# Xiongda337/fpm-OpenCV

Hardware: AMD Instinct MI355X
Metric: LED-updates/sec (patch·LED/s), 256² patch × 293 LEDs; 1/2/4/8 GPU (higher is better)
Workload: dtype f32

## Files before the change

### fpm-opencv_amd/csrc/fpm_fused.hip

```cpp
#include <hip/hip_runtime.h>

#include <vector>

#include "dft16.hpp"
#include "fft_lds.hpp"
#include "fpm_state.hpp"
#include "fused256.hpp"
#include "fused_common.hpp"
#include "fused_sync.hpp"
#include "launch.hpp"
#include "ledtab.hpp"
#include "tilemax.hpp"
#include "update.hpp"

namespace fpm {

constexpr int n_parts(int ks) { return ks == 1 ? 2 : ks; }
constexpr int part_cols(int ks) { return fz::NP / n_parts(ks); }

template <int NT>
struct FzCfg {
    static_assert(NT == 512, "512 threads per workgroup");
    static constexpr int NG = NT / 16;
    static constexpr int RPG = fz::NROWS / NG;
    static constexpr int NW = NT / 64;
    static constexpr int XT = XTILE;
};

template <int NT, int KS, bool GAIN>
__global__ void __launch_bounds__(NT, 1) k_fused_iteration(FusedArgs a) {
    using namespace fz;
    using C = FzCfg<NT>;
    constexpr int NG = C::NG, RPG = C::RPG, NW = C::NW;
    ClockProbe probe;
    probe.start();
    static_assert(KS == 1 || KS == 2 || KS == 4, "one workgroup per patch, or split mode with 2 / 4");
    static_assert(6 * RPG * 16 <= C::XT, "pupil numerators are parked in the group's exchange tile");
    constexpr int NPARTS = n_parts(KS), TH = part_cols(KS), TLD = TH + 1;
    extern __shared__ __attribute__((aligned(16))) float2 sm[];
    const int nrows = NROWS + a.n_tail_rows;
    float2 *scr_all = sm;
    float2 *th = scr_all + NG * C::XT;
    float2 *tw2 = th + (nrows + 2) * TLD;
    float2 *tw = tw2 + 256;
    float2 *tailX = tw + 256;
    float2 *tailF = tailX + MAXTAIL;
    float *red = (float *)(tailF + MAXTAIL);
    int *sig = (int *)(red + 48);
    int2 *tpx = (int2 *)(sig + 96);
    int *tky = (int *)(tpx + MAXTAIL);
    float *tmx = (float *)(tky + MAXTAILROWS);
    unsigned *dirty = (unsigned *)(tmx + a.band.nbt);
    int *ccnt = (int *)(dirty + ((a.band.nbt + 31) >> 5));

    const DevState &st = a.st;
    const int tid = threadIdx.x, g = tid >> 4, t = tid & 15, gg = (tid >> 4) & 3;
    const int xrd = exch_rbase(t);
    const int lane = tid & 63, w = tid >> 6;
    constexpr bool split = KS > 1;
    const int hown = split ? (int)((blockIdx.x >> 3) % KS) : -1;
    const int b = split ? (int)((blockIdx.x / (8 * KS)) * 8 + (blockIdx.x & 7)) : (int)blockIdx.x;
    if (b >= st.B) return;
    const int hb = hown < 0 ? 0 : hown, he = hown < 0 ? NPARTS : hown + 1;
    float2 *xch = split ? a.xch + (size_t)b * xch_patch_elems(KS) : nullptr;
    int *flg = split ? a.flags + KS * b : nullptr;
    int *xccs = split ? a.flags + KS * st.B + 1 + KS * b : nullptr;
    const int R = st.r, NB = st.nb, L = st.L;
    float2 *scr = scr_all + g * C::XT;
    const int nwords = (a.band.nbt + 31) >> 5;

    if (tid == 0) {
#pragma unroll
        for (int i = 0; i < MAXTAIL; ++i) tpx[i] = a.tail_px[i];
#pragma unroll
        for (int i = 0; i < MAXTAILROWS; ++i) tky[i] = a.tail_ky[i];
    }
    for (int i = tid; i < 256; i += NT) {
        tw[i] = a.tw[i];
        tw2[i] = a.tw[((i >> 4) * (i & 15)) & 255];
    }
    for (int i = tid; i < 96; i += NT) {
        const int ky = i - KYOFF;
        int s = -1;
        if (ky >= -R && ky <= R) {
            if (ky >= a.ky_lo && ky < a.ky_lo + a.n_fft_rows) s = ky - a.ky_lo;
#pragma unroll
            for (int q = 0; q < MAXTAILROWS; ++q)
                if (q < a.n_tail_rows && a.tail_ky[q] == ky) s = NROWS + q;
        }
        sig[i] = s;
    }
    auto band_dy = [&](int k) { return (int)(((float)k + 0.5f) * a.band.rnbx); };
    auto band_gtile = [&](int k) {
        const int dy = band_dy(k);
        return (a.band.bty0 + dy) * st.ntx + a.band.btx0 + (k - dy * a.band.nbx);
    };
    float *tmax_g = st.tmax + (size_t)b * st.ntx * st.nty;
    unsigned *dirty_g = st.tdirty + (size_t)b * ((st.ntx * st.nty + 31) / 32);
    for (int k = tid; k < a.band.nbt; k += NT) tmx[k] = tmax_g[band_gtile(k)];
    for (int i = tid; i < nwords; i += NT) dirty[i] = dirty_g[i];

    float2 *spec = st.spec + (size_t)b * L * L;
    float2 *pup = st.pupil + (size_t)b * NB * NB;
    int kyr[RPG];
    bool ron[RPG];
    float2 P[RPG][6];
    unsigned inmask[RPG];
#pragma unroll
    for (int j = 0; j < RPG; ++j) {
        kyr[j] = a.ky_lo + g + NG * j;
        ron[j] = g + NG * j < a.n_fft_rows;
        inmask[j] = 0;
#pragma unroll
        for (int s = 0; s < 6; ++s) {
            const int kx = slot_kx(t, s);
            const bool in = ron[j] && (kyr[j] * kyr[j] + kx * kx <= R * R);
            inmask[j] |= (in ? 1u : 0u) << s;
            P[j][s] = in ? pup[(kyr[j] + R) * NB + kx + R] : make_float2(0.f, 0.f);
        }
    }
    int2 *ltl = a.ledtab_off >= 0 ? (int2 *)((char *)sm + a.ledtab_off) : nullptr;
    const LedTab lt{ltl, a.order, a.x0, a.y0, NP / 2};
    if (ltl) lt.fill(ltl, a.n_order, tid, NT);
    __syncthreads();
    const int zoff = nrows * TLD;
    int roff[6];
#pragma unroll
    for (int s = 0; s < 6; ++s) {
        const int sg = sig[slot_kx(t, s) + KYOFF];
        roff[s] = sg >= 0 ? sg * TLD : zoff;
    }
    for (int i = tid; i < TLD; i += NT) th[zoff + i] = make_float2(0.f, 0.f);
    const bool towner = tid < a.n_tail_px;
    const int2 tp = towner ? tpx[tid] : make_int2(0, 0);
    float2 Pt = towner ? pup[(tp.x + R) * NB + tp.y + R] : make_float2(0.f, 0.f);
    float2 NPt = make_float2(0.f, 0.f), Ot = make_float2(0.f, 0.f);
    float pm = st.pmax[b];
    auto pm_of_red = [&]() {
        float pm2 = red[32];
#pragma unroll
        for (int i = 1; i < NW; ++i) pm2 = fmaxf(pm2, red[32 + i]);
        return sqrtf(pm2);
    };
    bool pupil_done = false;
    bool local = false;
    const __amdgpu_buffer_rsrc_t rx =
        __builtin_amdgcn_make_buffer_rsrc(xch, 0, split ? xch_patch_elems(KS) * (int)sizeof(float2) : 0, 0x00020000);
    const __amdgpu_buffer_rsrc_t rf = __builtin_amdgcn_make_buffer_rsrc(flg, 0, split ? KS * (int)sizeof(int) : 0, 0x00020000);
    const __amdgpu_buffer_rsrc_t rs =
        __builtin_amdgcn_make_buffer_rsrc(split ? st.spec + (size_t)b * L * L : nullptr, 0,
                                          split ? L * L * (int)sizeof(float2) : 0, 0x00020000);
    if (split) {
        if (tid == 0) {
            const int mine = xcc_id() + 1;
            __hip_atomic_store(xccs + hown, mine, __ATOMIC_RELAXED, __HIP_MEMORY_SCOPE_AGENT);
            bool same = true;
#pragma unroll
            for (int p = 0; p < KS; ++p) {
                if (p == hown) continue;
                int other = 0;
                for (int spins = 0; (other = __hip_atomic_load(xccs + p, __ATOMIC_RELAXED,
                                                               __HIP_MEMORY_SCOPE_AGENT)) == 0; ++spins) {
                    if (spins > (1 << 23) ||
                        __hip_atomic_load(a.abort_flag, __ATOMIC_RELAXED, __HIP_MEMORY_SCOPE_AGENT)) {
                        __hip_atomic_store(a.abort_flag, 1, __ATOMIC_RELAXED, __HIP_MEMORY_SCOPE_AGENT);
                        break;
                    }
                    __builtin_amdgcn_s_sleep(2);
                }
                same = same && other == mine;
            }
            ccnt[1] = same;
        }
        __syncthreads();
        local = ccnt[1] != 0;
        __syncthreads();
    }
    typedef unsigned u32x2_t __attribute__((ext_vector_type(2)));
    const int lane_off = tid * (int)sizeof(float2);
    auto xst = [&](int slot, float2 v) {
        const u32x2_t d = __builtin_bit_cast(u32x2_t, v);
        if (local) __builtin_amdgcn_raw_buffer_store_b64(d, rx, lane_off, slot * (int)sizeof(float2), 0);
        else __builtin_amdgcn_raw_buffer_store_b64(d, rx, lane_off, slot * (int)sizeof(float2), 16);
    };
    auto xld = [&](int slot) {
        return __builtin_bit_cast(
            float2, local ? __builtin_amdgcn_raw_buffer_load_b64(rx, lane_off, slot * (int)sizeof(float2), kAuxL2Volatile)
                          : __builtin_amdgcn_raw_buffer_load_b64(rx, lane_off, slot * (int)sizeof(float2),
                                                                 (int)(16u | (1u << 31))));
    };
    auto sst = [&](float2 *p, float2 v) {
        if (split && !local) {
            const int off = (int)((p - (st.spec + (size_t)b * L * L)) * (int)sizeof(float2));
            __builtin_amdgcn_raw_buffer_store_b64(__builtin_bit_cast(u32x2_t, v), rs, off, 0, 16);
        } else {
            *p = v;
        }
    };
    const float epsn = st.eps * (float)(NP * NP);
    const float epsn_im = st.eps_im * (float)(NP * NP);
    __syncthreads();

    FPM_STAMPS_BEGIN()
    auto window = [&](int itn) {
        const LedPos p = lt.at(itn);
        return spec + (unsigned)(p.yc * L + p.xc);
    };
    auto soff = [](int s) { return 16 * fz::SK[s] - (s >= 3 ? fz::NP : 0); };
    auto ldO = [&](const float2 *sr, int j, int s) {
        const float2 *lr = sr + (kyr[j] * L + t);
        return ((inmask[j] >> s) & 1) ? lr[soff(s)] : make_float2(0.f, 0.f);
    };
    float2 Opre[RPG][6];
    if (a.n_order > 0) {
        const float2 *sr = window(0);
#pragma unroll
        for (int j = 0; j < RPG; ++j)
#pragma unroll
            for (int s = 0; s < 6; ++s) Opre[j][s] = ldO(sr, j, s);
        if (towner) Ot = sr[tp.x * L + tp.y];
    }
    for (int it = 0; it < a.n_order; ++it) {
        const LedPos lp = lt.at(it);
        const int led = lp.led, xc = lp.xc, yc = lp.yc;
        float2 *srow = spec + (unsigned)(yc * L + xc);
        const uint16_t *Ib = a.meas + ((size_t)led * st.B + b) * NP * NP;
        const float gl = fused_gain<GAIN>(st, led, b);

        if (towner) tailX[tid] = pout(pmul(pin(Ot), pin(Pt)));
        __syncthreads();
        FPM_STAMP(0)

        float2 v[16], r[16];
        float2 F[RPG][6];
        bool aborted = false;
#pragma unroll 1
        for (int h = hb; h < he; ++h) {
            Tw wt;
            wt.load(tw2, t);
            constexpr int NBLK = TH / 4;
            auto colx = [&](int r8) { return (r8 & 15) + 16 * gg + 64 * (r8 >> 4); };
            auto ldI = [&](int xl, uint4 (&n)[2]) {
                const uint4 *ip = (const uint4 *)(Ib + ((xl + TH * h) * 16 + t) * 16);
#pragma unroll
                for (int i = 0; i < 2; ++i) n[i] = ld_stream(ip + i);
            };
            float2 X[RPG][6];
#pragma unroll
            for (int j = 0; j < RPG; ++j)
#pragma unroll
                for (int s = 0; s < 6; ++s) X[j][s] = pout(pmul(pin(Opre[j][s]), pin(P[j][s])));
#pragma unroll
            for (int j = 0; j < RPG; ++j) {
                if (!ron[j]) continue;
#pragma unroll
                for (int k = 0; k < 16; ++k) v[k] = make_float2(0.f, 0.f);
#pragma unroll
                for (int s = 0; s < 6; ++s) v[SK[s]] = X[j][s];
                idft256_in6(v, r, scr, wt, t, xrd);
                float2 *row = th + (g + NG * j) * TLD + t;
                if constexpr (NPARTS == 2) {
                    if (h == 0) {
#pragma unroll
                        for (int m = 0; m < 8; ++m) row[16 * m] = r[m];
                    } else {
#pragma unroll
                        for (int m = 0; m < 8; ++m) row[16 * m] = r[8 + m];
                    }
                } else {
                    if (h == 0) {
#pragma unroll
                        for (int m = 0; m < 4; ++m) row[16 * m] = r[m];
                    } else if (h == 1) {
#pragma unroll
                        for (int m = 0; m < 4; ++m) row[16 * m] = r[4 + m];
                    } else if (h == 2) {
#pragma unroll
                        for (int m = 0; m < 4; ++m) row[16 * m] = r[8 + m];
                    } else {
#pragma unroll
                        for (int m = 0; m < 4; ++m) row[16 * m] = r[12 + m];
                    }
                }
            }
            FPM_STAMP(7)
            for (int idx = tid; tid < NT / 2 && idx < a.n_tail_rows * TH; idx += NT / 2) {
                const int q = idx / TH, xl = idx - q * TH, x = xl + TH * h;
                const int p0 = a.tail_row_p0[q], np_ = a.tail_row_np[q];
                const int ti = (x * (a.tail_row_kx0[q] + NP)) & (NP - 1);
                pf2 wa = pin(tw[ti]), wb = pin(tw[(ti + x) & (NP - 1)]);
                const pf2 wstep = pin(tw[(2 * x) & (NP - 1)]);
                pf2 s2 = {0.f, 0.f}, s3 = {0.f, 0.f};
                int p = 0;
                for (; p + 1 < np_; p += 2) {
                    s2 += pmulc(pin(tailX[p0 + p]), wa);
                    s3 += pmulc(pin(tailX[p0 + p + 1]), wb);
                    wa = pmul(wa, wstep);
                    wb = pmul(wb, wstep);
                }
                if (p < np_) s2 += pmulc(pin(tailX[p0 + p]), wa);
                th[(NROWS + q) * TLD + xl] = pout(s2 + s3);
            }
            if (tid == 0) *ccnt = NW;
            __syncthreads();
            FPM_STAMP(1)

            float2 tin[6];
#pragma unroll
            for (int s = 0; s < 6; ++s) tin[s] = th[roff[s] + colx(w)];
            int r8 = w;
#pragma unroll 1
            for (;;) {
                const int xl = colx(r8);
                uint4 cI[2];
                int nx = 0;
                if (lane == 0) nx = atomicAdd(ccnt, 1);
                nx = __builtin_amdgcn_readfirstlane(nx);
                ldI(xl, cI);
#pragma unroll
                for (int k = 0; k < 16; ++k) v[k] = make_float2(0.f, 0.f);
#pragma unroll
                for (int s = 0; s < 6; ++s) v[SK[s]] = tin[s];
                idft256_in6(v, r, scr, wt, t, xrd);
                {
                    const int xn = colx(nx < NBLK ? nx : r8);
#pragma unroll
                    for (int s = 0; s < 6; ++s) tin[s] = th[roff[s] + xn];
                }
                const unsigned iw[8] = {cI[0].x, cI[0].y, cI[0].z, cI[0].w, cI[1].x, cI[1].y, cI[1].z, cI[1].w};
#pragma unroll
                for (int m2 = 0; m2 < 16; ++m2) {
                    const float Iv = (float)((m2 & 1) ? (iw[m2 >> 1] >> 16) : (iw[m2 >> 1] & 0xffffu));
                    const pf2 tt = pin(r[m2]) + (pf2){epsn, epsn_im};
                    const float mag2 = __builtin_fmaf(tt.x, tt.x, tt.y * tt.y);
                    const float sc = amp_scale(mag2, Iv);
                    v[m2] = pout(pin(r[m2]) * sc);
                }
                float2 o[6];
                dft256_out6(v, o, scr, wt, t, xrd);
#pragma unroll
                for (int s = 0; s < 6; ++s) th[roff[s] + (roff[s] == zoff ? TLD : 0) + xl] = o[s];
                if (nx >= NBLK) break;
                r8 = nx;
            }
            FPM_STAMP(10)
            __syncthreads();
            FPM_STAMP(2)

#pragma unroll
            for (int j = 0; j < RPG; ++j)
#pragma unroll
                for (int s = 0; s < 6; ++s) Opre[j][s] = ldO(srow, j, s);
#pragma unroll
            for (int j = 0; j < RPG; ++j) {
                if (!ron[j]) {
#pragma unroll
                    for (int s = 0; s < 6; ++s) F[j][s] = make_float2(0.f, 0.f);
                    continue;
                }
                float2 o[6];
                row_dft_part<NPARTS>(th + (g + NG * j) * TLD + t, v, o, scr, wt, t, xrd, h);
#pragma unroll
                for (int s = 0; s < 6; ++s) F[j][s] = h == hb ? o[s] : cadd(F[j][s], o[s]);
            }
            FPM_STAMP(8)
            for (int pp = g; g < NG / 2 && pp < a.n_tail_px; pp += NG / 2) {
                const int2 px = tpx[pp];
                const float2 *row = th + sig[px.x + KYOFF] * TLD;
                pf2 s2p = {0.f, 0.f};
                pf2 wk = pin(tw[((t + TH * h) * (px.y + NP)) & (NP - 1)]);
                const pf2 wstep = pin(tw[(16 * (px.y + NP)) & (NP - 1)]);
#pragma unroll
                for (int m = 0; m < TH / 16; ++m) {
                    s2p += pmul(pin(row[t + 16 * m]), wk);
                    if (m < TH / 16 - 1) wk = pmul(wk, wstep);
                }
                float2 s2 = pout(s2p);
                s2.x = row16_sum(s2.x);
                s2.y = row16_sum(s2.y);
                if (t == 0) tailF[pp] = h != hb ? cadd(tailF[pp], s2) : s2;
            }
            __syncthreads();
            FPM_STAMP(3)
        }
        if (split) {
            const int par = it & 1;
            const int mine = (hown * 2 + par) * kXchHalf;
            if (it < a.stall_led || a.stall_led < 0 || hown != KS - 1) {
#pragma unroll
                for (int j = 0; j < RPG; ++j)
#pragma unroll
                    for (int s = 0; s < 6; ++s)
                        if ((inmask[j] >> s) & 1) xst(mine + (j * 6 + s) * NT, F[j][s]);
                if (tid < a.n_tail_px) xst(mine + kXchTF, tailF[tid]);
                FPM_STAMP(11)
                handoff_publish(flg + hown, it + 1, local);
            }
            if (!handoff_wait<KS>(flg, hown, it + 1, a.abort_flag, ccnt + 1, local, rf)) {
                aborted = true;
                break;
            }
            FPM_STAMP(12)
            float2 ox[KS > 1 ? KS - 1 : 1][RPG][6];
#pragma unroll
            for (int q = 0; q < KS - 1; ++q) {
                const int pp = q < hown ? q : q + 1;
                const int base = (pp * 2 + par) * kXchHalf;
#pragma unroll
                for (int j = 0; j < RPG; ++j)
#pragma unroll
                    for (int s = 0; s < 6; ++s) {
                        const bool in = (inmask[j] >> s) & 1;
                        ox[q][j][s] = in ? xld(base + (j * 6 + s) * NT) : make_float2(0.f, 0.f);
                    }
            }
#pragma unroll
            for (int j = 0; j < RPG; ++j)
#pragma unroll
                for (int s = 0; s < 6; ++s) {
                    float2 acc = make_float2(0.f, 0.f);
#pragma unroll
                    for (int p = 0; p < KS; ++p) {
                        const float2 lo = ox[p < KS - 1 ? p : KS - 2][j][s], hi = ox[p > 0 ? p - 1 : 0][j][s];
                        const float2 o = p == hown ? F[j][s] : p < hown ? lo : hi;
                        acc = p == 0 ? o : cadd(acc, o);
                    }
                    F[j][s] = acc;
                }
            if (tid < a.n_tail_px) {
                float2 acc = make_float2(0.f, 0.f);
#pragma unroll
                for (int p = 0; p < KS; ++p) {
                    const float2 o = p == hown ? tailF[tid] : xld(((p * 2 + par) * kXchHalf) + kXchTF);
                    acc = p == 0 ? o : cadd(acc, o);
                }
                tailF[tid] = acc;
            }
        }

        unsigned *tmu = (unsigned *)tmx;
        auto note = [&](int py, int px, float ao, float an) {
            const int ti = ((py >> 4) - a.band.bty0) * a.band.nbx + ((px >> 4) - a.band.btx0);
            const unsigned cur = tmu[ti];
            if (an < ao && cur <= __float_as_uint(ao)) atomicOr(&dirty[ti >> 5], 1u << (ti & 31));
            if (__float_as_uint(an) > cur) atomicMax(&tmu[ti], __float_as_uint(an));
        };
        if (it > 0) pm = pm_of_red();
#pragma unroll
        for (int j = 0; j < RPG; ++j)
#pragma unroll
            for (int s = 0; s < 6; ++s) {
                float2 num = make_float2(0.f, 0.f);
                if ((inmask[j] >> s) & 1) {
                    float oa;
                    const float2 nv = slot_update<GAIN>(F[j][s], Opre[j][s], P[j][s], pm, gl, st, num, oa);
                    sst(srow + (kyr[j] * L + t) + soff(s), nv);
                    note(yc + kyr[j], xc + slot_kx(t, s), oa, cmag(nv));
                }
                scr[(j * 6 + s) * 16 + t] = num;
            }
        if (towner) {
            float oa;
            const float2 nv = slot_update<GAIN>(tailF[tid], Ot, Pt, pm, gl, st, NPt, oa);
            sst(srow + tp.x * L + tp.y, nv);
            note(yc + tp.x, xc + tp.y, oa, cmag(nv));
        }
        FPM_STAMP(9)
        __syncthreads();
        if (it + 1 < a.n_order) {
            const float2 *sr = window(it + 1);
#pragma unroll
            for (int j = 0; j < RPG; ++j)
#pragma unroll
                for (int s = 0; s < 6; ++s) Opre[j][s] = ldO(sr, j, s);
            if (towner) Ot = sr[tp.x * L + tp.y];
        }
        FPM_STAMP(4)

        float cm = 0.f, dm = 0.f;
        for (int k = tid; k < a.band.nbt; k += NT) {
            const bool d = tile_dirty(dirty, k);
            if (d) dm = fmaxf(dm, tmx[k]);
            else cm = fmaxf(cm, tmx[k]);
        }
        cm = wave_max_nonneg(cm);
        dm = wave_max_nonneg(dm);
        if (lane == 0) {
            red[w] = cm;
            red[16 + w] = dm;
        }
        __syncthreads();
        cm = red[0];
        dm = red[16];
#pragma unroll
        for (int i = 1; i < NW; ++i) {
            cm = fmaxf(cm, red[i]);
            dm = fmaxf(dm, red[16 + i]);
        }
        float omax = cm;
        if (dm > cm) {
            for (int k = w; k < a.band.nbt; k += NW) {
                if (!tile_dirty(dirty, k) || !(tmx[k] > cm)) continue;
                const int ty = a.band.bty0 + band_dy(k), tx = a.band.btx0 + k - band_dy(k) * a.band.nbx;
                float2 e[4];
#pragma unroll
                for (int jj = 0; jj < 4; ++jj) {
                    const int pp = lane + 64 * jj;
                    e[jj] = spec[(unsigned)((ty * 16 + (pp >> 4)) * L + tx * 16 + (pp & 15))];
                }
                float mm = 0.f;
#pragma unroll
                for (int jj = 0; jj < 4; ++jj) mm = fmaxf(mm, cmag(e[jj]));
                mm = wave_max_nonneg(mm);
                if (lane == 0) {
                    tmx[k] = mm;
                    atomicAnd(&dirty[k >> 5], ~(1u << (k & 31)));
                }
            }
            __syncthreads();
            float m2 = 0.f;
            for (int k = tid; k < a.band.nbt; k += NT)
                if (!tile_dirty(dirty, k)) m2 = fmaxf(m2, tmx[k]);
            m2 = wave_max_nonneg(m2);
            __syncthreads();
            if (lane == 0) red[w] = m2;
            __syncthreads();
            omax = red[0];
#pragma unroll
            for (int i = 1; i < NW; ++i) omax = fmaxf(omax, red[i]);
        }
        FPM_STAMP(5)
        const float rom = 1.0f / omax;
        float pmx = 0.f;
#pragma unroll
        for (int j = 0; j < RPG; ++j)
#pragma unroll
            for (int s = 0; s < 6; ++s) {
                const float2 n = scr[(j * 6 + s) * 16 + t];
                P[j][s] = make_float2(P[j][s].x + n.x * rom, P[j][s].y + n.y * rom);
                pmx = fmaxf(pmx, cabs2(P[j][s]));
            }
        if (towner) {
            Pt = make_float2(Pt.x + NPt.x * rom, Pt.y + NPt.y * rom);
            pmx = fmaxf(pmx, cabs2(Pt));
        }
        pmx = wave_max_nonneg(pmx);
        if (lane == 0) red[32 + w] = pmx;
        pupil_done = true;
        FPM_STAMP(6)
        (void)aborted;
    }
    __syncthreads();
    probe.stop(a.st.clk);
    if (pupil_done) pm = pm_of_red();
    if (a.dbg && (split ? (tid == 0 && (hown == 0 || hown == KS - 1)) : (tid == 0 || tid == NT - 64)))
        for (int i = 0; i < kStamps; ++i) atomicAdd(&a.dbg[((split ? hown : tid) ? kStamps : 0) + i], acc[i]);
    if (hown > 0) return;

#pragma unroll
    for (int j = 0; j < RPG; ++j)
#pragma unroll
        for (int s = 0; s < 6; ++s)
            if ((inmask[j] >> s) & 1) pup[(kyr[j] + R) * NB + slot_kx(t, s) + R] = P[j][s];
    if (towner) pup[(tp.x + R) * NB + tp.y + R] = Pt;
    for (int k = tid; k < a.band.nbt; k += NT) tmax_g[band_gtile(k)] = tmx[k];
    for (int i = tid; i < nwords; i += NT) dirty_g[i] = dirty[i];
    if (tid == 0) st.pmax[b] = pm;
}

namespace {
size_t fused_lds_bytes(int ks, int nbt, int n_tail_rows) {
    const int tld = part_cols(ks) + 1;
    return (size_t)(32 * XTILE + (fz::NROWS + n_tail_rows + 2) * tld + 512 + 2 * fz::MAXTAIL) * sizeof(float2) +
           48 * sizeof(float) + 96 * sizeof(int) + fz::MAXTAIL * sizeof(int2) + fz::MAXTAILROWS * sizeof(int) +
           (size_t)nbt * sizeof(float) + (size_t)(nbt + 31) / 32 * sizeof(unsigned) + 2 * sizeof(int);
}

}

int fused_threads(int np, int r, int L, const DevState &st) {
    const FusedGeom g = fused_geometry(np, r);
    if (!g.ok || L % kTile != 0) return 0;
    if (!band_valid(st)) return 0;
    return fused_lds_bytes(1, band_of(st).nbt, g.n_tail_rows) <= kLdsCap ? 512 : 0;
}

size_t fused_T_elems(int, int, int) { return 1; }

size_t fused_xch_elems(int B, int ks) { return (size_t)B * xch_patch_elems(ks); }
size_t fused_flag_words(int B, int ks) { return 2 * (size_t)ks * B + 1; }

int fused_split_parts(int nt, int B, int n_cu, const Switches &sw) {
    if (nt != 512 || B < 1 || sw.no_split) return 1;
    auto fits = [&](int ks) { return 8 * ks * ((B + 7) / 8) <= n_cu; };
    if (sw.split >= 0) {
        const int ks = sw.split;
        return (ks == 2 || ks == 4) && fits(ks) ? ks : 1;
    }
    return fits(4) ? 4 : fits(2) ? 2 : 1;
}

hipError_t launch_fused_iteration(const DevState &st, const FusedLaunch &in, int ks, float2 *xch, int *flags,
                                  int stall_led, hipStream_t s) {
    const FusedGeom g = fused_geometry(st.np, st.r);
    if (!g.ok) return hipErrorInvalidValue;
    if (ks != 1 && ((ks != 2 && ks != 4) || !xch || !flags)) return hipErrorInvalidValue;
    if (!band_valid(st)) return hipErrorInvalidValue;
    FusedArgs a{};
    fill_np256_args(a, st, g, in);
    a.xch = ks > 1 ? xch : nullptr;
    a.flags = ks > 1 ? flags : nullptr;
    a.abort_flag = ks > 1 ? flags + ks * st.B : nullptr;
    a.stall_led = ks > 1 ? stall_led : -1;
    const size_t lds0 = fused_lds_bytes(ks, a.band.nbt, g.n_tail_rows);
    if (lds0 > kLdsCap) return hipErrorInvalidValue;
    size_t lds;
    a.ledtab_off = ledtab_offset(lds0, in.n_order, st.L, kLdsCap, lds, in.no_ledtab);
    if (in.gains) {
        if (ks == 1) return launch_lds(k_fused_iteration<512, 1, true>, st.B, 512, lds, &a, s);
        return launch_np256_parts(ks == 4 ? k_fused_iteration<512, 4, true> : k_fused_iteration<512, 2, true>, ks, lds, &a,
                                  s);
    }
    if (ks == 1) return launch_lds(k_fused_iteration<512, 1, false>, st.B, 512, lds, &a, s);
    return launch_np256_parts(ks == 4 ? k_fused_iteration<512, 4, false> : k_fused_iteration<512, 2, false>, ks, lds, &a,
                              s);
}

}
```

### fpm-opencv_amd/csrc/fused256.hpp

```cpp
#pragma once
#include <hip/hip_runtime.h>

#include "cpk.hpp"
#include "dft16.hpp"

namespace fpm {

template <int N>
__device__ __forceinline__ void to_pk(const float2 (&a)[N], pf2 (&p)[N]) {
#pragma unroll
    for (int i = 0; i < N; ++i) p[i] = pin(a[i]);
}
template <int N>
__device__ __forceinline__ void from_pk(const pf2 (&p)[N], float2 (&a)[N]) {
#pragma unroll
    for (int i = 0; i < N; ++i) a[i] = pout(p[i]);
}

template <bool INV>
__device__ __forceinline__ void pdft16_in6(const pf2 (&in)[16], pf2 (&r)[16]) {
    const pf2 a0 = in[0], b1 = in[1], b13 = in[13], c2 = in[2], c14 = in[14], d15 = in[15];
    pf2 v[16];
    v[0] = a0; v[4] = a0; v[8] = a0; v[12] = a0;
    v[1] = b1 + b13;
    v[5] = psub_w4<INV>(b1, b13);
    v[9] = b1 - b13;
    v[13] = padd_w4<INV>(b1, b13);
    v[2] = c2 + c14;
    v[6] = psub_w4<INV>(c2, c14);
    v[10] = c2 - c14;
    v[14] = padd_w4<INV>(c2, c14);
    const pf2 z = {0.f, 0.f};
    v[3] = d15;
    v[7] = psub_w4<INV>(z, d15);
    v[11] = -d15;
    v[15] = padd_w4<INV>(z, d15);
    pmid_tw<INV>(v);
    pstage2<INV>(v);
#pragma unroll
    for (int m = 0; m < 16; ++m) r[m] = v[4 * (m & 3) + (m >> 2)];
}

template <bool INV>
__device__ __forceinline__ void pdft16_out6(pf2 (&v)[16], pf2 (&o)[6]) {
#pragma unroll
    for (int k1 = 0; k1 < 4; ++k1) pbf4<INV>(v[k1], v[k1 + 4], v[k1 + 8], v[k1 + 12]);
    pmid_tw<INV>(v);
    o[0] = (v[0] + v[2]) + (v[1] + v[3]);
    o[1] = (v[4] + v[6]) + (v[5] + v[7]);
    o[2] = padd_w4<INV>(v[8], v[10]) + (v[9] + v[11]);
    o[3] = psub_w4<INV>(v[4] - v[6], v[5] - v[7]);
    o[4] = psub_w4<INV>(psub_w4<INV>(v[8], v[10]), v[9] - v[11]);
    o[5] = psub_w4<INV>(v[12] - v[14], v[13] - v[15]);
}

template <bool INV, int H>
__device__ __forceinline__ void pdft16_inhalf(pf2 (&v)[16], pf2 (&r)[16]) {
#pragma unroll
    for (int k1 = 0; k1 < 4; ++k1) {
        if (H == 0) {
            const pf2 a0 = v[k1], a1 = v[k1 + 4];
            v[k1] = a0 + a1;
            v[k1 + 4] = padd_w4<INV>(a0, a1);
            v[k1 + 8] = a0 - a1;
            v[k1 + 12] = psub_w4<INV>(a0, a1);
        } else {
            const pf2 a2 = v[k1 + 8], a3 = v[k1 + 12];
            v[k1] = a2 + a3;
            v[k1 + 4] = -padd_w4<INV>(a2, a3);
            v[k1 + 8] = a2 - a3;
            v[k1 + 12] = -psub_w4<INV>(a2, a3);
        }
    }
    pmid_tw<INV>(v);
    pstage2<INV>(v);
#pragma unroll
    for (int m = 0; m < 16; ++m) r[m] = v[4 * (m & 3) + (m >> 2)];
}

template <bool INV, int Q>
__device__ __forceinline__ void pbf4_one(pf2 a, pf2 &y0, pf2 &y1, pf2 &y2, pf2 &y3) {
    const pf2 z = {0.f, 0.f};
    if constexpr (Q == 0) {
        y0 = a; y1 = a; y2 = a; y3 = a;
    } else if constexpr (Q == 1) {
        y0 = a; y1 = padd_w4<INV>(z, a); y2 = -a; y3 = psub_w4<INV>(z, a);
    } else if constexpr (Q == 2) {
        y0 = a; y1 = -a; y2 = a; y3 = -a;
    } else {
        y0 = a; y1 = psub_w4<INV>(z, a); y2 = -a; y3 = padd_w4<INV>(z, a);
    }
}

template <bool INV, int Q>
__device__ __forceinline__ void pdft16_inquarter(pf2 (&v)[16], pf2 (&r)[16]) {
#pragma unroll
    for (int k1 = 0; k1 < 4; ++k1) {
        const pf2 a = v[k1 + 4 * Q];
        pbf4_one<INV, Q>(a, v[k1], v[k1 + 4], v[k1 + 8], v[k1 + 12]);
    }
    pmid_tw<INV>(v);
    pstage2<INV>(v);
#pragma unroll
    for (int m = 0; m < 16; ++m) r[m] = v[4 * (m & 3) + (m >> 2)];
}

struct Tw {
    float2 w[16];
    __device__ __forceinline__ void load(const float2 *tw2, int t) {
#pragma unroll
        for (int m = 0; m < 16; ++m) w[m] = tw2[m * 16 + t];
    }
    __device__ __forceinline__ float2 operator[](int m) const { return w[m]; }
};

template <class TW>
__device__ __forceinline__ void idft256_in6(float2 (&v)[16], float2 (&r)[16], float2 *scr, const TW &wt, int t,
                                            int xrd) {
    pf2 pv[16], py[16];
    to_pk(v, pv);
    pdft16_in6<true>(pv, py);
    ptwiddle15<true>(py, wt);
    float2 y[16];
    from_pk(py, y);
    exchange16(scr, t, xrd, y, v);
    to_pk(v, pv);
    pdft16<true>(pv, py);
    from_pk(py, r);
}

template <class TW>
__device__ __forceinline__ void dft256_out6(float2 (&v)[16], float2 (&o)[6], float2 *scr, const TW &wt, int t,
                                            int xrd) {
    pf2 pv[16], py[16], po[6];
    to_pk(v, pv);
    pdft16<false>(pv, py);
    ptwiddle15<false>(py, wt);
    float2 y[16];
    from_pk(py, y);
    exchange16(scr, t, xrd, y, v);
    to_pk(v, pv);
    pdft16_out6<false>(pv, po);
    from_pk(po, o);
}

template <int H, class TW>
__device__ __forceinline__ void dft256_inhalf_out6(float2 (&v)[16], float2 (&o)[6], float2 *scr, const TW &wt, int t,
                                                   int xrd) {
    pf2 pv[16], py[16], po[6];
    to_pk(v, pv);
    pdft16_inhalf<false, H>(pv, py);
    ptwiddle15<false>(py, wt);
    float2 y[16];
    from_pk(py, y);
    exchange16(scr, t, xrd, y, v);
    to_pk(v, pv);
    pdft16_out6<false>(pv, po);
    from_pk(po, o);
}

template <int NPARTS, int P, class TW>
__device__ __forceinline__ void dft256_inpart_out6(float2 (&v)[16], float2 (&o)[6], float2 *scr, const TW &wt,
                                                   int t, int xrd) {
    if constexpr (NPARTS == 2) {
        dft256_inhalf_out6<P>(v, o, scr, wt, t, xrd);
    } else {
        static_assert(NPARTS == 4, "two or four column parts");
        pf2 pv[16], py[16], po[6];
        to_pk(v, pv);
        pdft16_inquarter<false, P>(pv, py);
        ptwiddle15<false>(py, wt);
        float2 y[16];
        from_pk(py, y);
        exchange16(scr, t, xrd, y, v);
        to_pk(v, pv);
        pdft16_out6<false>(pv, po);
        from_pk(po, o);
    }
}

template <int NPARTS, class TW, int HH = 0>
__device__ __forceinline__ void row_dft_part(const float2 *row, float2 (&v)[16], float2 (&o)[6], float2 *scr,
                                             const TW &wt, int t, int xrd, int h) {
    constexpr int MPP = 16 / NPARTS;
    if constexpr (HH < NPARTS) {
        if (HH == h) {
#pragma unroll
            for (int k = 0; k < 16; ++k) v[k] = make_float2(0.f, 0.f);
#pragma unroll
            for (int m = 0; m < MPP; ++m) v[HH * MPP + m] = row[16 * m];
            dft256_inpart_out6<NPARTS, HH>(v, o, scr, wt, t, xrd);
        } else {
            row_dft_part<NPARTS, TW, HH + 1>(row, v, o, scr, wt, t, xrd, h);
        }
    }
}

}
```

Before: 7.382 million.

## Process two rows per group jointly in half-split row DFTs

In the two-part split mode, each 16-thread group now handles its two rows together. It computes only the needed half of each row's first radix-16 stage and packs both rows into one 256-point exchange, in both the inverse and forward directions. This halves the LDS exchanges and second-stage DFTs per row pair, and it changes the column mapping for intensity loads and the tail paths to an interleaved 8-column layout. In exchange the indexing is more complex, the twiddle loads are per half, and the pair path assumes RPG==2.

```diff
diff --git a/fpm-opencv_amd/csrc/fpm_fused.hip b/fpm-opencv_amd/csrc/fpm_fused.hip
--- a/fpm-opencv_amd/csrc/fpm_fused.hip
+++ b/fpm-opencv_amd/csrc/fpm_fused.hip
@@ -25,6 +25,7 @@
     static constexpr int RPG = fz::NROWS / NG;
     static constexpr int NW = NT / 64;
     static constexpr int XT = XTILE;
+    static __device__ __forceinline__ int row(int g, int j) { return g + NG * j; }
 };
 
 template <int NT, int KS, bool GAIN>
@@ -37,6 +38,8 @@
     static_assert(KS == 1 || KS == 2 || KS == 4, "one workgroup per patch, or split mode with 2 / 4");
     static_assert(6 * RPG * 16 <= C::XT, "pupil numerators are parked in the group's exchange tile");
     constexpr int NPARTS = n_parts(KS), TH = part_cols(KS), TLD = TH + 1;
+    constexpr bool PAIR = NPARTS == 2;
+    static_assert(!PAIR || RPG == 2, "a row pair per group");
     extern __shared__ __attribute__((aligned(16))) float2 sm[];
     const int nrows = NROWS + a.n_tail_rows;
     float2 *scr_all = sm;
@@ -108,8 +111,8 @@
     unsigned inmask[RPG];
 #pragma unroll
     for (int j = 0; j < RPG; ++j) {
-        kyr[j] = a.ky_lo + g + NG * j;
-        ron[j] = g + NG * j < a.n_fft_rows;
+        kyr[j] = a.ky_lo + C::row(g, j);
+        ron[j] = C::row(g, j) < a.n_fft_rows;
         inmask[j] = 0;
 #pragma unroll
         for (int s = 0; s < 6; ++s) {
@@ -131,6 +134,9 @@
         roff[s] = sg >= 0 ? sg * TLD : zoff;
     }
     for (int i = tid; i < TLD; i += NT) th[zoff + i] = make_float2(0.f, 0.f);
+    const int pj = t >> 3;
+    const bool pon = pj ? ron[RPG - 1] : ron[0];
+    const int prow = (pon ? C::row(g, pj) * TLD : zoff) + (t & 7);
     const bool towner = tid < a.n_tail_px;
     const int2 tp = towner ? tpx[tid] : make_int2(0, 0);
     float2 Pt = towner ? pup[(tp.x + R) * NB + tp.y + R] : make_float2(0.f, 0.f);
@@ -240,8 +246,9 @@
             wt.load(tw2, t);
             constexpr int NBLK = TH / 4;
             auto colx = [&](int r8) { return (r8 & 15) + 16 * gg + 64 * (r8 >> 4); };
+            auto xcol = [&](int xl) { return PAIR ? 8 * h + (xl & 7) + 16 * (xl >> 3) : xl + TH * h; };
             auto ldI = [&](int xl, uint4 (&n)[2]) {
-                const uint4 *ip = (const uint4 *)(Ib + ((xl + TH * h) * 16 + t) * 16);
+                const uint4 *ip = (const uint4 *)(Ib + (xcol(xl) * 16 + t) * 16);
 #pragma unroll
                 for (int i = 0; i < 2; ++i) n[i] = ld_stream(ip + i);
             };
@@ -250,24 +257,23 @@
             for (int j = 0; j < RPG; ++j)
 #pragma unroll
                 for (int s = 0; s < 6; ++s) X[j][s] = pout(pmul(pin(Opre[j][s]), pin(P[j][s])));
-#pragma unroll
-            for (int j = 0; j < RPG; ++j) {
-                if (!ron[j]) continue;
-#pragma unroll
-                for (int k = 0; k < 16; ++k) v[k] = make_float2(0.f, 0.f);
-#pragma unroll
-                for (int s = 0; s < 6; ++s) v[SK[s]] = X[j][s];
-                idft256_in6(v, r, scr, wt, t, xrd);
-                float2 *row = th + (g + NG * j) * TLD + t;
-                if constexpr (NPARTS == 2) {
-                    if (h == 0) {
-#pragma unroll
-                        for (int m = 0; m < 8; ++m) row[16 * m] = r[m];
-                    } else {
-#pragma unroll
-                        for (int m = 0; m < 8; ++m) row[16 * m] = r[8 + m];
-                    }
-                } else {
+            if constexpr (PAIR) {
+                if (ron[0]) {
+                    idft256_pair_in6(X, v, r, scr, wt, t, xrd, h);
+                    float2 *row = th + prow + (pon ? 0 : TLD);
+#pragma unroll
+                    for (int m = 0; m < 16; ++m) row[8 * m] = r[m];
+                }
+            } else {
+#pragma unroll
+                for (int j = 0; j < RPG; ++j) {
+                    if (!ron[j]) continue;
+#pragma unroll
+                    for (int k = 0; k < 16; ++k) v[k] = make_float2(0.f, 0.f);
+#pragma unroll
+                    for (int s = 0; s < 6; ++s) v[SK[s]] = X[j][s];
+                    idft256_in6(v, r, scr, wt, t, xrd);
+                    float2 *row = th + C::row(g, j) * TLD + t;
                     if (h == 0) {
 #pragma unroll
                         for (int m = 0; m < 4; ++m) row[16 * m] = r[m];
@@ -285,7 +291,7 @@
             }
             FPM_STAMP(7)
             for (int idx = tid; tid < NT / 2 && idx < a.n_tail_rows * TH; idx += NT / 2) {
-                const int q = idx / TH, xl = idx - q * TH, x = xl + TH * h;
+                const int q = idx / TH, xl = idx - q * TH, x = xcol(xl);
                 const int p0 = a.tail_row_p0[q], np_ = a.tail_row_np[q];
                 const int ti = (x * (a.tail_row_kx0[q] + NP)) & (NP - 1);
                 pf2 wa = pin(tw[ti]), wb = pin(tw[(ti + x) & (NP - 1)]);
@@ -351,25 +357,44 @@
             for (int j = 0; j < RPG; ++j)
 #pragma unroll
                 for (int s = 0; s < 6; ++s) Opre[j][s] = ldO(srow, j, s);
-#pragma unroll
-            for (int j = 0; j < RPG; ++j) {
-                if (!ron[j]) {
-#pragma unroll
-                    for (int s = 0; s < 6; ++s) F[j][s] = make_float2(0.f, 0.f);
-                    continue;
-                }
-                float2 o[6];
-                row_dft_part<NPARTS>(th + (g + NG * j) * TLD + t, v, o, scr, wt, t, xrd, h);
-#pragma unroll
-                for (int s = 0; s < 6; ++s) F[j][s] = h == hb ? o[s] : cadd(F[j][s], o[s]);
+            if constexpr (PAIR) {
+                if (ron[0]) {
+                    wt.load(tw2, 8 * h + (t & 7));
+#pragma unroll
+                    for (int m = 0; m < 16; ++m) v[m] = th[prow + 8 * m];
+                    float2 o[RPG][6];
+                    dft256_pair_out6(v, o, scr, wt, t, xrd, h);
+#pragma unroll
+                    for (int j = 0; j < RPG; ++j)
+#pragma unroll
+                        for (int s = 0; s < 6; ++s) F[j][s] = h == hb ? o[j][s] : cadd(F[j][s], o[j][s]);
+                } else {
+#pragma unroll
+                    for (int j = 0; j < RPG; ++j)
+#pragma unroll
+                        for (int s = 0; s < 6; ++s) F[j][s] = make_float2(0.f, 0.f);
+                }
+            } else {
+#pragma unroll
+                for (int j = 0; j < RPG; ++j) {
+                    if (!ron[j]) {
+#pragma unroll
+                        for (int s = 0; s < 6; ++s) F[j][s] = make_float2(0.f, 0.f);
+                        continue;
+                    }
+                    float2 o[6];
+                    row_dft_part<NPARTS>(th + C::row(g, j) * TLD + t, v, o, scr, wt, t, xrd, h);
+#pragma unroll
+                    for (int s = 0; s < 6; ++s) F[j][s] = h == hb ? o[s] : cadd(F[j][s], o[s]);
+                }
             }
             FPM_STAMP(8)
             for (int pp = g; g < NG / 2 && pp < a.n_tail_px; pp += NG / 2) {
                 const int2 px = tpx[pp];
                 const float2 *row = th + sig[px.x + KYOFF] * TLD;
                 pf2 s2p = {0.f, 0.f};
-                pf2 wk = pin(tw[((t + TH * h) * (px.y + NP)) & (NP - 1)]);
-                const pf2 wstep = pin(tw[(16 * (px.y + NP)) & (NP - 1)]);
+                pf2 wk = pin(tw[(xcol(t) * (px.y + NP)) & (NP - 1)]);
+                const pf2 wstep = pin(tw[((PAIR ? 32 : 16) * (px.y + NP)) & (NP - 1)]);
 #pragma unroll
                 for (int m = 0; m < TH / 16; ++m) {
                     s2p += pmul(pin(row[t + 16 * m]), wk);
diff --git a/fpm-opencv_amd/csrc/fused256.hpp b/fpm-opencv_amd/csrc/fused256.hpp
--- a/fpm-opencv_amd/csrc/fused256.hpp
+++ b/fpm-opencv_amd/csrc/fused256.hpp
@@ -54,30 +54,6 @@
     o[5] = psub_w4<INV>(v[12] - v[14], v[13] - v[15]);
 }
 
-template <bool INV, int H>
-__device__ __forceinline__ void pdft16_inhalf(pf2 (&v)[16], pf2 (&r)[16]) {
-#pragma unroll
-    for (int k1 = 0; k1 < 4; ++k1) {
-        if (H == 0) {
-            const pf2 a0 = v[k1], a1 = v[k1 + 4];
-            v[k1] = a0 + a1;
-            v[k1 + 4] = padd_w4<INV>(a0, a1);
-            v[k1 + 8] = a0 - a1;
-            v[k1 + 12] = psub_w4<INV>(a0, a1);
-        } else {
-            const pf2 a2 = v[k1 + 8], a3 = v[k1 + 12];
-            v[k1] = a2 + a3;
-            v[k1 + 4] = -padd_w4<INV>(a2, a3);
-            v[k1 + 8] = a2 - a3;
-            v[k1 + 12] = -psub_w4<INV>(a2, a3);
-        }
-    }
-    pmid_tw<INV>(v);
-    pstage2<INV>(v);
-#pragma unroll
-    for (int m = 0; m < 16; ++m) r[m] = v[4 * (m & 3) + (m >> 2)];
-}
-
 template <bool INV, int Q>
 __device__ __forceinline__ void pbf4_one(pf2 a, pf2 &y0, pf2 &y1, pf2 &y2, pf2 &y3) {
     const pf2 z = {0.f, 0.f};
@@ -144,39 +120,20 @@
     from_pk(po, o);
 }
 
-template <int H, class TW>
-__device__ __forceinline__ void dft256_inhalf_out6(float2 (&v)[16], float2 (&o)[6], float2 *scr, const TW &wt, int t,
-                                                   int xrd) {
-    pf2 pv[16], py[16], po[6];
-    to_pk(v, pv);
-    pdft16_inhalf<false, H>(pv, py);
-    ptwiddle15<false>(py, wt);
-    float2 y[16];
-    from_pk(py, y);
-    exchange16(scr, t, xrd, y, v);
-    to_pk(v, pv);
-    pdft16_out6<false>(pv, po);
-    from_pk(po, o);
-}
-
 template <int NPARTS, int P, class TW>
 __device__ __forceinline__ void dft256_inpart_out6(float2 (&v)[16], float2 (&o)[6], float2 *scr, const TW &wt,
                                                    int t, int xrd) {
-    if constexpr (NPARTS == 2) {
-        dft256_inhalf_out6<P>(v, o, scr, wt, t, xrd);
-    } else {
-        static_assert(NPARTS == 4, "two or four column parts");
-        pf2 pv[16], py[16], po[6];
-        to_pk(v, pv);
-        pdft16_inquarter<false, P>(pv, py);
-        ptwiddle15<false>(py, wt);
-        float2 y[16];
-        from_pk(py, y);
-        exchange16(scr, t, xrd, y, v);
-        to_pk(v, pv);
-        pdft16_out6<false>(pv, po);
-        from_pk(po, o);
-    }
+    static_assert(NPARTS == 4, "four column parts (two halves run as row pairs, below)");
+    pf2 pv[16], py[16], po[6];
+    to_pk(v, pv);
+    pdft16_inquarter<false, P>(pv, py);
+    ptwiddle15<false>(py, wt);
+    float2 y[16];
+    from_pk(py, y);
+    exchange16(scr, t, xrd, y, v);
+    to_pk(v, pv);
+    pdft16_out6<false>(pv, po);
+    from_pk(po, o);
 }
 
 template <int NPARTS, class TW, int HH = 0>
@@ -196,4 +153,131 @@
     }
 }
 
-}
+
+template <bool INV, int H, bool W2>
+__device__ __forceinline__ void pbf4_half(pf2 a0, pf2 a1, pf2 a2, pf2 a3, pf2 &lo, pf2 &hi) {
+    const pf2 s02 = W2 ? padd_w4<INV>(a0, a2) : a0 + a2, d02 = W2 ? psub_w4<INV>(a0, a2) : a0 - a2;
+    const pf2 s13 = a1 + a3, e13 = a1 - a3;
+    if constexpr (H == 0) {
+        lo = s02 + s13;
+        hi = padd_w4<INV>(d02, e13);
+    } else {
+        lo = s02 - s13;
+        hi = psub_w4<INV>(d02, e13);
+    }
+}
+
+template <bool INV, int H>
+__device__ __forceinline__ void pdft16_in6_outhalf(const pf2 (&in)[6], pf2 (&r)[8]) {
+    const pf2 a0 = in[0], b1 = in[1], c2 = in[2], b13 = in[3], c14 = in[4], d15 = in[5];
+    const pf2 z = {0.f, 0.f};
+    pf2 v[16];
+    v[0] = a0; v[4] = a0; v[8] = a0; v[12] = a0;
+    v[1] = b1 + b13;
+    v[5] = psub_w4<INV>(b1, b13);
+    v[9] = b1 - b13;
+    v[13] = padd_w4<INV>(b1, b13);
+    v[2] = c2 + c14;
+    v[6] = psub_w4<INV>(c2, c14);
+    v[10] = c2 - c14;
+    v[14] = padd_w4<INV>(c2, c14);
+    v[3] = d15;
+    v[7] = psub_w4<INV>(z, d15);
+    v[11] = -d15;
+    v[15] = padd_w4<INV>(z, d15);
+    pmid_tw<INV>(v);
+    pbf4_half<INV, H, false>(v[0], v[1], v[2], v[3], r[0], r[4]);
+    pbf4_half<INV, H, false>(v[4], v[5], v[6], v[7], r[1], r[5]);
+    pbf4_half<INV, H, true>(v[8], v[9], v[10], v[11], r[2], r[6]);
+    pbf4_half<INV, H, false>(v[12], v[13], v[14], v[15], r[3], r[7]);
+}
+
+template <bool INV, int H>
+__device__ __forceinline__ void pdft16_inhalf_out6(const pf2 (&in)[8], pf2 (&o)[6]) {
+    pf2 v[16];
+#pragma unroll
+    for (int k1 = 0; k1 < 4; ++k1) {
+        const pf2 a = in[k1], b = in[k1 + 4];
+        if (H == 0) {
+            v[k1] = a + b;
+            v[k1 + 4] = padd_w4<INV>(a, b);
+            v[k1 + 8] = a - b;
+            v[k1 + 12] = psub_w4<INV>(a, b);
+        } else {
+            v[k1] = a + b;
+            v[k1 + 4] = -padd_w4<INV>(a, b);
+            v[k1 + 8] = a - b;
+            v[k1 + 12] = -psub_w4<INV>(a, b);
+        }
+    }
+    pmid_tw<INV>(v);
+    o[0] = (v[0] + v[2]) + (v[1] + v[3]);
+    o[1] = (v[4] + v[6]) + (v[5] + v[7]);
+    o[2] = padd_w4<INV>(v[8], v[10]) + (v[9] + v[11]);
+    o[3] = psub_w4<INV>(v[4] - v[6], v[5] - v[7]);
+    o[4] = psub_w4<INV>(psub_w4<INV>(v[8], v[10]), v[9] - v[11]);
+    o[5] = psub_w4<INV>(v[12] - v[14], v[13] - v[15]);
+}
+
+template <int H, class TW>
+__device__ __forceinline__ void idft256_pair_stage1(const float2 (&X)[2][6], pf2 (&py)[16], const TW &wt) {
+#pragma unroll
+    for (int j = 0; j < 2; ++j) {
+        pf2 in[6], o[8];
+        to_pk(X[j], in);
+        pdft16_in6_outhalf<true, H>(in, o);
+#pragma unroll
+        for (int i = 0; i < 8; ++i) py[8 * j + i] = o[i];
+    }
+    pf2 w[8];
+#pragma unroll
+    for (int i = 0; i < 8; ++i) w[i] = pin(wt[8 * H + i]);
+#pragma unroll
+    for (int j = 0; j < 2; ++j) {
+        if constexpr (H == 0) {
+            ptw_block<true, 4>(&py[8 * j + 1], &w[1]);
+            ptw_block<true, 3>(&py[8 * j + 5], &w[5]);
+        } else {
+            ptw_block<true, 4>(&py[8 * j], &w[0]);
+            ptw_block<true, 4>(&py[8 * j + 4], &w[4]);
+        }
+    }
+}
+
+template <class TW>
+__device__ __forceinline__ void idft256_pair_in6(const float2 (&X)[2][6], float2 (&v)[16], float2 (&r)[16], float2 *scr,
+                                                 const TW &wt, int t, int xrd, int h) {
+    pf2 pv[16], py[16];
+    if (h == 0) idft256_pair_stage1<0>(X, py, wt);
+    else idft256_pair_stage1<1>(X, py, wt);
+    float2 y[16];
+    from_pk(py, y);
+    exchange16(scr, t, xrd, y, v);
+    to_pk(v, pv);
+    pdft16<true>(pv, py);
+    from_pk(py, r);
+}
+
+template <class TW>
+__device__ __forceinline__ void dft256_pair_out6(float2 (&v)[16], float2 (&o)[2][6], float2 *scr, const TW &wx, int t,
+                                                 int xrd, int h) {
+    pf2 pv[16], py[16];
+    to_pk(v, pv);
+    pdft16<false>(pv, py);
+    ptwiddle15<false>(py, wx);
+    float2 y[16];
+    from_pk(py, y);
+    exchange16(scr, t, xrd, y, v);
+    to_pk(v, pv);
+#pragma unroll
+    for (int j = 0; j < 2; ++j) {
+        pf2 in[8], po[6];
+#pragma unroll
+        for (int i = 0; i < 8; ++i) in[i] = pv[8 * j + i];
+        if (h == 0) pdft16_inhalf_out6<false, 0>(in, po);
+        else pdft16_inhalf_out6<false, 1>(in, po);
+        from_pk(po, o[j]);
+    }
+}
+
+}
```

After: 7.752 million (median of 6 runs). 5.0% higher.
